# nsdumont/Semantic-Spiking-Neural-SLAM-2023

Hardware: AMD Instinct MI355X
Metric: sim-sec/wall-sec, SSP-SLAM ssp_dim=1015 10k PI neurons, 1/2/4/8 MI355X (higher is better)
Workload: dtype f32; 1 GPU; PathIntegration 2-D ssp_dim=1015 pi_n_neurons=10000/VCO (508 VCOs, 5080000 LIF neurons), configs[1]; eval_points_per_vco=4000, parallelism=1 GPU, build_cache=miss

## Files before the change

### include/ssn.h

```cpp
#ifndef SSN_H
#define SSN_H

#include <stdint.h>

#ifdef __cplusplus
extern "C" {
#endif

#define SSN_ABI_VERSION 10

enum ssn_status {
  SSN_OK = 0,
  SSN_EINVAL = -1,
  SSN_EHIP = -2,
  SSN_ERCCL = -3,
  SSN_ENOMEM = -4,
  SSN_EUNSUPPORTED = -5
};

enum ssn_dtype { SSN_F32 = 0, SSN_F64 = 1 };
enum ssn_buffer_kind { SSN_BUF_REAL = 0, SSN_BUF_I32 = 1, SSN_BUF_TAPS = 2 ,
                       SSN_BUF_DRIVES = 3  };
enum ssn_neuron { SSN_LIF = 0, SSN_LIFRATE = 1, SSN_RELU = 2 };

// ... 167 lines not shown

enum ssn_probe_kind {
  SSN_PROBE_PK_FMA = 0, SSN_PROBE_PK_MUL = 1, SSN_PROBE_PK_ADD = 2,
  SSN_PROBE_TRANS = 3,
  SSN_PROBE_FMA = 4, SSN_PROBE_ADD = 5,
  SSN_PROBE_DPP = 6, SSN_PROBE_MOV = 7, SSN_PROBE_READLANE = 8,
  SSN_PROBE_CNDMASK = 9, SSN_PROBE_OTHER = 10,
  SSN_PROBE_N_KINDS = 11
};
int ssn_probe_issue_rate(int32_t device, int32_t kind, int32_t waves_per_simd, int32_t iters,
                         double* ns_per_wave_instruction, double* shader_mhz);

int ssn_get_counters(ssn_sim* sim, ssn_counters* out);
int ssn_get_kernel_times(ssn_sim* sim, ssn_kernel_time* out, int32_t capacity);
int64_t ssn_n_steps(ssn_sim* sim);
int ssn_device_count(void);
const char* ssn_last_error(void);
const char* ssn_version(void);

#ifdef __cplusplus
}
#endif
#endif
```

### semantic-spiking-neural-slam-2023_amd/_lib.py

```python
import ctypes as C
import os

_HERE = os.path.dirname(os.path.abspath(__file__))
LIB_PATH = os.environ.get("SSN_HIP_LIB") or os.path.join(_HERE, "libssn_hip.so")

SSN_ABI_VERSION = 10
SSN_F32, SSN_F64 = 0, 1
SSN_BUF_REAL, SSN_BUF_I32, SSN_BUF_TAPS, SSN_BUF_DRIVES = 0, 1, 2, 3
NEURON_CODE = {"lif": 0, "lifrate": 1, "relu": 2}
OP_CODE = {"fill": 1, "table": 2, "axpy": 3, "matvec": 4, "lowpass": 5, "ensarray": 6, "neurons": 7,
           "pes": 8, "voja": 9, "cleanup": 10, "gate": 11, "lincomb": 12}
SSN_PLAN_NO_FUSED_CORE = 1
SSN_PLAN_NO_LIF_FAST = 2
SSN_PLAN_DENSE_DECODERS = 4
SSN_PLAN_NO_SPMV = 8
SSN_PLAN_SEPARATE_FINISH = 16
SSN_PLAN_NO_BLOCK_KERNEL = 128
SSN_PLAN_NO_FFT = 512
SSN_PLAN_SPMV_OWN_LIST = 1024
SSN_PLAN_NO_ITEM_BATCH = 4096
SSN_PLAN_ENS_PARTIALS = 8192
SSN_PLAN_NO_STAGE_BATCH = 262144
SSN_PLAN_NO_FACTORED_GRID = 524288
SSN_PLAN_NO_ROUNDS = 2097152
# ... 79 lines not shown
    "ssn_read_signal": (C.c_int, [C.c_void_p, C.c_int64, C.c_int64, C.c_void_p]),
    "ssn_write_signal": (C.c_int, [C.c_void_p, C.c_int64, C.c_int64, C.c_void_p]),
    "ssn_read_buffer": (C.c_int, [C.c_void_p, C.c_int32, C.c_void_p, C.c_int64]),
    "ssn_write_buffer": (C.c_int, [C.c_void_p, C.c_int32, C.c_void_p, C.c_int64]),
    "ssn_run_phase": (C.c_int, [C.c_void_p, C.c_int32]),
    "ssn_exchange_size": (C.c_int64, [C.c_void_p]),
    "ssn_cycle_steps": (C.c_int64, [C.c_void_p]),
    "ssn_exchange_pack": (C.c_int, [C.c_void_p, C.c_void_p]),
    "ssn_exchange_unpack": (C.c_int, [C.c_void_p, C.c_void_p]),
    "ssn_phase_async": (C.c_int, [C.c_void_p, C.c_int32, C.c_void_p, C.c_void_p]),
    "ssn_phase_sync": (C.c_int, [C.c_void_p, C.c_void_p]),
    "ssn_probe_issue_rate": (C.c_int, [C.c_int32, C.c_int32, C.c_int32, C.c_int32, C.POINTER(C.c_double), C.POINTER(C.c_double)]),
    "ssn_get_counters": (C.c_int, [C.c_void_p, C.POINTER(Counters)]),
    "ssn_get_kernel_times": (C.c_int, [C.c_void_p, C.POINTER(KernelTime), C.c_int32]),
    "ssn_n_steps": (C.c_int64, [C.c_void_p]),
    "ssn_device_count": (C.c_int, []),
    "ssn_last_error": (C.c_char_p, []),
    "ssn_version": (C.c_char_p, []),
}

_lib = None


def load():
    global _lib
    if _lib is not None:
        return _lib
    if not os.path.exists(LIB_PATH):
        raise ImportError(f"{LIB_PATH} not found: build it with `python -c 'import __graft_entry__ as g; g.build()'` "
                          "or `make -C semantic-spiking-neural-slam-2023_amd/csrc` (there is no CPU fallback)")
# ... 15 lines not shown
```

### semantic-spiking-neural-slam-2023_amd/csrc/ssn_host.hip

```cpp
#include <hip/hip_runtime.h>
#include <dlfcn.h>
#include <algorithm>
#include <climits>
#include <cmath>
#include <cstdarg>
#include <cstdio>
#include <cstdlib>
#include <cstring>
#include <memory>
#include <mutex>
#include <map>
#include <set>
#include <string>
#include <thread>
#include <vector>

#include "../../include/ssn.h"
#include "ssn_launch.hpp"

namespace {

__global__ void k_set_block(ssn::StepCtx* ctx, long long block_start) { ctx->block_start = block_start; }
__global__ void k_advance(ssn::StepCtx* ctx, long long n) { ctx->step += n; }

thread_local std::string g_err;

int fail(int code, const char* fmt, ...) {
  char buf[1024];
  va_list ap;
  va_start(ap, fmt);
  vsnprintf(buf, sizeof buf, fmt, ap);
  va_end(ap);
  g_err = buf;
  return code;
}

}
// ... 92 lines not shown
  X(REAL, lat_solo, "SSN_LAT_SOLO", 3.0, "balancer: latency of a gate / argmax body (us)")                                                        \
  X(OFF0, pes_fold, "SSN_PES_FOLD", true, "fold the filter of a PES rule's activities into the rule's body")                                      \
  X(ON1, phased_pes_fold, "SSN_PHASED_PES_FOLD", false, "... also in neuron-sharded plans")                                                       \
  X(OFF0, fuse_neurons, "SSN_FUSE_NEURONS", true, "neuron update of a dense population in the epilogue of its encoder product")                   \
  X(INT, fuse_min_rows, "SSN_FUSE_MIN_ROWS", 4097, "smallest population that is fused so (tests lower it)")                                       \
  X(OFF0, solo_chains, "SSN_SOLO_CHAINS", true, "serial chains of single-workgroup operators (RK_SOLO)")                                          \
  X(OFF0, phased_solo, "SSN_PHASED_SOLO", true, "... in neuron-sharded plans")                                                                    \
  X(ON1, solo_dft, "SSN_SOLO_DFT", false, "transforms as members of serial chains (measured slower)")                                             \
  X(REAL, solo_cap_us, "SSN_SOLO_CAP_US", 16.0, "longest serial chain in estimated microseconds")                                                 \
  X(LL, solo_max_len, "SSN_SOLO_MAX_LEN", 2048, "longest glue operator (elements) a single workgroup takes")                                      \
  X(OFF0, round_interleave, "SSN_ROUND_INTERLEAVE", true, "interleaved dispatch of a round's big grids behind its latency-bound head")            \
  X(OFF0, head_prio, "SSN_HEAD_PRIO", true, "raised wave priority for the head blocks of a round")                                                \
  X(PRESENT, phase2_sequential, "SSN_PHASE2_SEQUENTIAL", false, "sharded: phase 1 of a timestep and phase 0 of the next as two sets of rounds")   \
  X(INT, cycle_steps, "SSN_CYCLE_STEPS", 16, "sharded: timesteps pipelined over the exchange (2..64; 0 or 1: off)")                               \
  X(PRESENT, no_batch_reorder, "SSN_NO_BATCH_REORDER", false, "time-batched stages keep the builder's operator order")                            \
  X(PRESENT, no_zero_skip, "SSN_NO_ZERO_SKIP", false, "time-batched products are multiplied out even when their whole input is zero")

struct PlanOptions {
  struct Int3 { int v[3] = {0, 0, 0}; };
  static constexpr int UNSET = INT_MIN;
  enum Kind { K_PRESENT, K_OFF0, K_ON1, K_INT, K_LL, K_REAL, K_INT3 };
  typedef bool T_PRESENT; typedef bool T_OFF0; typedef bool T_ON1; typedef int T_INT; typedef long long T_LL; typedef double T_REAL; typedef Int3 T_INT3;

  int flags = 0;
#define X(kind, name, env, def, doc) T_##kind name = def;
  SSN_PLAN_KNOBS(X)
#undef X

  bool has(int bit) const { return (flags & bit) != 0; }

  static PlanOptions read(int flags) {
// ... 76 lines not shown
  virtual int reserve_probes(int64_t n) = 0;
  virtual int run_steps(int64_t n, int profile) = 0;
  virtual int run_phase(int phase) = 0;
  virtual int64_t exchange_size() = 0;
  virtual int64_t cycle_len() = 0;
  virtual int exchange_copy(void* buf, bool pack) = 0;
  virtual int phase_async(int phase, void* buf, hipStream_t ext) = 0;
  virtual int phase_sync(hipStream_t ext) = 0;
  virtual int read_probe(int id, double* dst, void* dst_dev, int64_t first, int64_t count) = 0;
  virtual int64_t probe_count(int id) = 0;
  virtual int rw_signal(int64_t off, int64_t count, double* dst, const double* src) = 0;
  virtual int rw_buffer(int id, double* dst, const double* src, int64_t count) = 0;
  virtual int counters(ssn_counters* out) = 0;
  virtual int kernel_times(ssn_kernel_time* out, int capacity) = 0;
  virtual int64_t n_steps() = 0;
};

namespace {

template <typename T>
struct Sim final : ssn_sim {
  using MOp = ssn::MicroOp<T>;
  static constexpr int VW = 16 / sizeof(T);

  struct TapSet;
  struct DriveSet;
  struct Item {
    int type = IT_PROGRAM;
    int op_begin = 0, op_count = 0;
    ssn::EnsArgs<T> ens;
// ... 22 lines not shown
  hipStream_t stream = nullptr;
  hipStream_t copy_stream = nullptr;
  double* up_stage = nullptr;
  int64_t up_cap = 0;
  void* dl_stage = nullptr;
  int64_t dl_cap = 0;
  std::mutex dl_mutex;
  int64_t n_sig = 0;
  T* sig = nullptr;
  std::vector<double> sig_init;
  std::vector<Buf> bufs;
  std::vector<Item> items;
  std::vector<void*> owned;
  T* bsig = nullptr;
  int block = 0;
  bool core_empty = false;
  const PlanOptions opt;
  bool fused_core = false;
  bool fused_defer = false;
  ssn::FinishArgs<T> fin_begin, fin_flush;
  bool fused_block = false;
  ssn::BlockArgs<T> blk;
  struct TapSet { std::vector<ssn_tap_desc> list; int* d_tab = nullptr; double amp = 0.0; };
  std::map<int, TapSet> tap_sets;
  struct DriveSet { ssn_drive_desc rec; std::vector<int32_t> src; int* d_tab = nullptr; int* d_tab_rows = nullptr; };
  std::map<int, DriveSet> drive_sets;
  std::set<int> sparse_w;
  std::set<int> learned_w;
  std::vector<std::pair<int64_t, std::pair<int*, int*>>> spike_lists;
  std::vector<int64_t> seg_spikes;
// ... 540 lines not shown
    }
    pslots.assign(m->n_probes, ssn::ProbeSlot{nullptr, 1, 0, 0});
    probe_store.resize((size_t)m->n_probes);
    for (int i = 0; i < m->n_probes; ++i) pslots[i].every = probes[i].every;
    CHK(dupload(&d_pslots, pslots));
    exchange.assign(m->exchange, m->exchange + (m->n_exchange > 0 ? m->n_exchange : 0));
    phased = !exchange.empty();
    for (auto& r : exchange) CHK(check_range(r.lo, r.hi - r.lo, "exchange"));
    bool has_batched_stage = false;
    for (int i = 0; i < m->n_ops; ++i) has_batched_stage = has_batched_stage || m->ops[i].stage != 1;
    for (auto& p : probes) has_batched_stage = has_batched_stage || p.stage != 1;
    batched_mask.assign((size_t)n_sig, 0);
    if (has_batched_stage && phased) return fail(SSN_EINVAL, "a neuron-sharded model is stepped whole (build it unstaged)");
    if (has_batched_stage) {
      block = m->block_steps > 0 ? m->block_steps : ((int64_t)1025 * n_sig * (int64_t)sizeof(T) <= (256ll << 20) ? 1024 : 256);
      CHK(dmalloc(&bsig, (int64_t)(block + 1) * n_sig * (int64_t)sizeof(T)));
      CHK(init_bsig());
      pre_to_core.assign(m->pre_to_core, m->pre_to_core + m->n_pre_to_core);
      core_to_post.assign(m->core_to_post, m->core_to_post + m->n_core_to_post);
      for (auto& r : pre_to_core) CHK(check_range(r.lo, r.hi - r.lo, "pre->core boundary"));
      for (auto& r : core_to_post) CHK(check_range(r.lo, r.hi - r.lo, "core->post boundary"));
    }
    steps_per_graph = m->steps_per_graph != 0 ? m->steps_per_graph : ((block == 0 || block % 64 == 0) ? 64 : 16);
    if (steps_per_graph > 128) return fail(SSN_EINVAL, "steps_per_graph %d: at most 128 (a glue block carries its timestep offset in 8 signed bits)", steps_per_graph);
    CHK(drive_tables());
    CHK(plan(m));
    CHK(capture());
    HIPCHK(hipStreamSynchronize(stream));
    return SSN_OK;
  }

  ssn::NeuronParams<T> neuron_params(int64_t type, const double* f) const {
// ... 418 lines not shown
      if (hipGetDeviceProperties(&prop, device) == hipSuccess) n_cu = prop.multiProcessorCount;
      if (opt.block_split_cus != PlanOptions::UNSET) n_cu = opt.block_split_cus;
      const int64_t n_ens = eo.i[2];
      for (int cand : {4, 2}) {
        if (K * cand <= n_cu && n_ens / cand >= 1024) { split_P = cand; break; }
      }
      { const int q = opt.block_split; if (q == 1 || q == 2 || q == 4 || q == 8) split_P = q; }
      if (split_P > 1) n_member = (int)(((n_ens + split_P - 1) / split_P + 3) / 4 * 4);
    }
    if (defer && !drv && !opt.has(SSN_PLAN_NO_BLOCK_KERNEL) && ens_fast(eo) && (sizeof(T) == 8 || (dt <= 0.05 * eo.f[0] && eo.f[1] >= dt)) &&
        ssn::ens_block_supported<T>((int)din, (int)dout, split_P > 1 ? n_member : (int)eo.i[2], opt.block_variant.v, &blk_threads, &blk_tpb, &blk_npt, &blk_lds)) {
      FilterTabs ft;
      CHK(filter_tables(ft, true));
      ssn::EnsArgs<T> ea;
      fill_ens_args(eo, taps, drv, ea);
      blk = ssn::BlockArgs<T>{};
      blk.enc = ea.enc; blk.bias = ea.bias; blk.dec = ea.dec; blk.S = ea.V;
      blk.xrows = bsig; blk.bsig = bsig; blk.sig = sig; blk.sig_w = sig;
      blk.didx = (const int*)bufs[eo.i[8]].d; blk.lp_state = ft.lp; blk.lp_a = ft.a; blk.lp_b = ft.b;
      blk.xrow = ft.xrow; blk.xalpha = ft.xalpha; blk.rowout = ft.ro;
      blk.n_sig = n_sig; blk.x_off = eo.i[0];
      blk.K = ea.K; blk.n = ea.n; blk.n_pad = ea.n_pad; blk.din = ea.din; blk.dout = ea.dout;
      blk.B = 0; blk.row0 = 1; blk.threads = blk_threads; blk.tpb = blk_tpb; blk.npt = blk_npt; blk.enc_lds = blk_lds;
      blk.dec_neuron_major = ea.fast == 1 ? 1 : 0;
      blk.np = ea.np;
      blk.P = split_P; blk.n_member = n_member; blk.xslots = nullptr; blk.xerr = nullptr;
      {
        unsigned long long* d_ss = nullptr;
        CHK(dzeros(&d_ss, 2));
        blk.slot_stats = d_ss;
// ... 367 lines not shown
    bool first_probe = true;
    for (size_t p = 0; p < probes.size(); ++p) {
      if (probes[p].stage != 1) {
        ssn::BatchOp<T> b{};
        b.bsig = bsig; b.n_sig = n_sig; b.kind = ssn::M_PROBE; b.src = probes[p].src; b.len = probes[p].width; b.p0 = d_pslots + p;
        post_ops.push_back(b);
        continue;
      }
      MOp op{};
      op.kind = ssn::M_PROBE; op.src = probes[p].src; op.len = probes[p].width; op.p0 = d_pslots + p;
      push_micro(op, -2, first_probe);
      first_probe = false;
    }
    optimise_batch(pre_ops);
    optimise_batch(post_ops);
    if (!fused) {
      MOp end{};
      end.kind = ssn::M_STEP_END;
      push_micro(end, -3, false);
    }
    force_barrier = true;
    flush();
    for (auto& it : items) if (it.phase < 0) it.phase = cur_phase;
    if (phased && cur_phase != 1) return fail(SSN_EINVAL, "a model with exchange ranges needs operators of phase 1");
    if (best_item >= 0) {
      items[best_item].dominant = true;
      const ssn::EnsArgs<T>& a = items[best_item].ens;
      dom_units = (int64_t)a.K * a.n;
      dom_bytes = (double)dom_units * (a.din + a.dout + 5) * sizeof(T);
    }
// ... 1104 lines not shown
      if (it.type == IT_PROGRAM) {
        for (const MOp& op : programs[(size_t)item_prog[(size_t)prog_i]]) micro_access(acc[i], op);
        ++prog_i;
      } else if (it.type == IT_VECOPS) {
        for (const MOp& op : vecops_host) micro_access(acc[i], op);
      } else {
        item_access(acc[i], it);
      }
    }
    item_deps.assign(items.size(), {});
    for (size_t i = 0; i < items.size(); ++i)
      for (size_t j = 0; j < i; ++j)
        if (hazard(acc[i], acc[j])) item_deps[i].push_back((int)j);
  }

  int init_bsig() {
    if (!bsig) return SSN_OK;
    CHK(upload(sig_init.data(), bsig, 1, n_sig, n_sig));
    for (int r = 1; r <= block; ++r)
      HIPCHK(hipMemcpyAsync(bsig + (size_t)r * n_sig, bsig, (size_t)n_sig * sizeof(T), hipMemcpyDeviceToDevice, stream));
    HIPCHK(hipStreamSynchronize(stream));
    return SSN_OK;
  }

  static bool batch_elementwise(const ssn::BatchOp<T>& o) { return kind_is(o.kind, MK_BATCH_EW); }
  static bool batch_writes(const ssn::BatchOp<T>& o) { return kind_is(o.kind, MK_BATCH_W); }
  static bool batch_reads(const ssn::BatchOp<T>& o) { return kind_is(o.kind, MK_BATCH_R); }
  static long long batch_read_len(const ssn::BatchOp<T>& o) { return kind_is(o.kind, MK_BATCH_PRODUCT) ? o.cols : o.len; }
  static int batch_hazard(const ssn::BatchOp<T>& a, const ssn::BatchOp<T>& b) {
    auto ov = [](long long x, long long xl, long long y, long long yl) { return x < y + yl && y < x + xl; };
    int kind = 0;
    auto pair = [&](long long x, long long xl, long long y, long long yl, bool prev) {
      if (!ov(x, xl, y, yl)) return;
      kind = std::max(kind, (x == y && !prev) ? 1 : 2);
    };
// ... 53 lines not shown
      if (!out.empty() && level[k] == last_level && o.kind == ssn::M_LOWPASS && out.back().kind == ssn::M_LOWPASS && out.back().a == o.a && out.back().b == o.b &&
          out.back().src_prev == o.src_prev && out.back().dst + out.back().len == o.dst && out.back().src + out.back().len == o.src) {
        out.back().len += o.len;
        continue;
      }
      out.push_back(o);
      last_level = level[k];
    }
    if (opt.debug_plan) {
      fprintf(stderr, "[ssn] time-batched stage: %zu operators -> %zu\n", ops.size(), out.size());
      for (const Op& o : out) fprintf(stderr, "[ssn]   batch op kind %d dst %lld src %lld len %lld cols %d prev %d\n", o.kind, (long long)o.dst, (long long)o.src, (long long)o.len, o.cols, o.src_prev);
    }
    ops.swap(out);
  }

  hipError_t run_batch(std::vector<ssn::BatchOp<T>>& ops, int B, int64_t step0) {
    auto elementwise = [](const ssn::BatchOp<T>& o) { return batch_elementwise(o); };
    std::vector<char> zero((size_t)n_sig, 0);
    const bool track = !opt.no_zero_skip;
    auto all_zero = [&](long long lo, long long n) { for (long long q = lo; q < lo + n; ++q) if (!zero[(size_t)q]) return false; return n > 0; };
    auto set_zero = [&](long long lo, long long n, bool v) { for (long long q = lo; q < lo + n; ++q) zero[(size_t)q] = v ? 1 : 0; };
    auto note = [&](const ssn::BatchOp<T>& o) {
      if (!track) return;
      switch (o.kind) {
        case ssn::M_TABLE: {
          bool z = false;
          for (size_t id = 0; id < table_dst.size() && id < table_idx_host.size(); ++id)
            if (table_dst[id].second > 0 && table_dst[id].first == o.dst && table_dst[id].second == o.len) z = table_is_zero((int)id, B, step0);
          set_zero(o.dst, o.len, z); break;
        }
        case ssn::M_FILL: set_zero(o.dst, o.len, o.a == T(0)); break;
        case ssn::M_AXPY_SET: set_zero(o.dst, o.len, !o.src_prev && all_zero(o.src, o.len)); break;
        case ssn::M_AXPY_INC: if (o.src_prev || !all_zero(o.src, o.len)) set_zero(o.dst, o.len, false); break;
        case ssn::M_PROBE: break;
        default: set_zero(o.dst, o.len, false); break;
      }
    };
    for (size_t i = 0; i < ops.size();) {
      ops[i].B = B; ops[i].step0 = step0;
      if (elementwise(ops[i]) && !opt.has(SSN_PLAN_NO_STAGE_BATCH)) {
        ssn::BatchOpList<T> l{};
        l.op[0] = ops[i];
        l.count = 1;
        size_t j = i + 1;
        for (; j < ops.size() && l.count < ssn::MAX_BATCH_OPS && elementwise(ops[j]); ++j) {
          ops[j].B = B; ops[j].step0 = step0;
          bool clash = false;
          for (int q = 0; q < l.count; ++q) clash = clash || batch_hazard(l.op[q], ops[j]) == 2;
          if (clash) break;
          l.op[l.count++] = ops[j];
        }
        if (l.count > 1) {
          hipError_t e = ssn::launch_batch_elementwise<T>(stream, l);
          if (e != hipSuccess) return e;
          for (int q = 0; q < l.count; ++q) note(l.op[q]);
          i = j;
          continue;
        }
      }
      if (track && kind_is(ops[i].kind, MK_BATCH_PRODUCT) && !ops[i].src_prev && all_zero(ops[i].src, ops[i].cols)) {
        ++batch_skipped;
        if (ops[i].kind == ssn::M_MATVEC_SET) {
          hipError_t e = hipMemset2DAsync(bsig + n_sig + ops[i].dst, (size_t)n_sig * sizeof(T), 0, (size_t)ops[i].len * sizeof(T), (size_t)B, stream);
          if (e != hipSuccess) return e;
          set_zero(ops[i].dst, ops[i].len, true);
        }
        ++i;
        continue;
      }
      hipError_t e = ssn::launch_batch_op<T>(stream, ops[i]);
      if (e != hipSuccess) return e;
      note(ops[i]);
      ++i;
    }
    return hipSuccess;
  }

  bool table_is_zero(int id, int B, int64_t step0) const {
    const ssn::TableSlot& t = tables[(size_t)id];
    const std::vector<int32_t>& ix = table_idx_host[(size_t)id];
    for (int64_t st = step0; st < step0 + B; ++st) {
      const int64_t rel = st - t.first_step;
      if (rel >= 0 && rel < (int64_t)ix.size() && ix[(size_t)rel] >= 0) return false;
    }
    return true;
  }
// ... 322 lines not shown
    Timing tm;
    tm.level = profile;
    if (profile) {
      const size_t per_step = profile == 2 ? items.size() + (round_mode ? launch_list.size() : 0) : (size_t)std::max(1, n_dom);
      const size_t need = fused_block ? (size_t)(2 * (n / std::max(1, block) + 2)) : (size_t)(2 * n * (int)per_step);
      if (need > 400000) return fail(SSN_EINVAL, "profile run too long (%lld steps): at most 200000 timed launches", (long long)n);
      while (ev_pool.size() < need) {
        hipEvent_t ev;
        HIPCHK(hipEventCreate(&ev));
        ev_pool.push_back(ev);
      }
    }
    HIPCHK(hipEventRecord(ev_run0, stream));
    int64_t done = 0;
    while (done < n) {
      const int64_t B = bsig ? std::min<int64_t>(block, n - done) : (n - done);
      const int64_t step0 = steps_done + done;
      if (bsig) {
        hipLaunchKernelGGL(k_set_block, dim3(1), dim3(1), 0, stream, d_ctx, (long long)step0);
        HIPCHK(hipGetLastError());
        HIPCHK(run_batch(pre_ops, (int)B, step0));
      }
      if (fused_defer) HIPCHK(ssn::launch_ens_finish<T>(stream, fin_begin));
      if (fused_block) {
        const bool timed = profile && B == block && tm.used + 2 <= ev_pool.size();
        blk.B = (int)B;
        if (blk.P > 1)
          HIPCHK(hipMemsetD32Async((hipDeviceptr_t)blk.xslots, (int)ssn::BLOCK_XCHG_SENTINEL, (size_t)3 * blk.K * 64, stream));
        if (timed) HIPCHK(hipEventRecord(ev_pool[tm.used], stream));
        HIPCHK(ssn::launch_ens_block<T>(stream, blk));
        if (timed) { HIPCHK(hipEventRecord(ev_pool[tm.used + 1], stream)); tm.used += 2; }
        HIPCHK(advance_clock(B));
      } else if (core_empty) {
        HIPCHK(advance_clock(B));
      } else if (profile) {
        int64_t s = 0;
        if (profile == 2 && round_mode && !graph_list.empty())
          for (; s + steps_per_graph <= B; s += steps_per_graph) {
            HIPCHK(launch_seq(graph_list, &tm));
            HIPCHK(advance_clock(steps_per_graph));
          }
        for (; s < B; ++s) {
          HIPCHK(launch_seq(launch_list, &tm));
          if (fused_defer) HIPCHK(advance_clock(1));
        }
      } else {
        int64_t left = B;
        if (step_graph.exec)
          for (; left >= steps_per_graph; left -= steps_per_graph) HIPCHK(hipGraphLaunch(step_graph.exec, stream));
        if (left > 0) HIPCHK(launch_steps((int)left, true));
      }
      if (fused_defer) HIPCHK(ssn::launch_ens_finish<T>(stream, fin_flush));
      if (bsig) {
        HIPCHK(run_batch(post_ops, (int)B, step0));
        HIPCHK(hipMemcpyAsync(bsig, bsig + (size_t)B * n_sig, (size_t)n_sig * sizeof(T), hipMemcpyDeviceToDevice, stream));
      }
      done += B;
    }
    HIPCHK(hipEventRecord(ev_run1, stream));
    HIPCHK(hipStreamSynchronize(stream));
    for (size_t j = 0; j < tm.used; j += 2) {
      float ms = 0.f;
      HIPCHK(hipEventElapsedTime(&ms, ev_pool[j], ev_pool[j + 1]));
      if (profile == 2) {
        const int ty = tm.types[j / 2];
        type_ms[ty] += ms;
        type_launches[ty] += 1;
        if (item_ms.size() != items.size() + round_launches.size()) { item_ms.assign(items.size() + round_launches.size(), 0.0); item_n.assign(items.size() + round_launches.size(), 0); }
        item_ms[(size_t)tm.items[j / 2]] += ms; item_n[(size_t)tm.items[j / 2]] += 1;
        continue;
      }
      dom_ms += ms;
// ... 208 lines not shown
                                              "k_argmax_partial", "k_round", "", "", ""};
    int n = 0;
    for (int t = 0; t < N_ITEM_TYPES; ++t) {
      if (!type_launches[t]) continue;
      if (n < capacity) {
        snprintf(out[n].name, sizeof out[n].name, "%s", names[t]);
        out[n].launches = type_launches[t];
        out[n].ms_total = type_ms[t];
      }
      ++n;
    }
    return n;
  }

  int64_t n_steps() override { return steps_done; }
};

template <typename T>
int create_sim(const ssn_model_desc* desc, ssn_sim** out) {
  auto s = std::make_unique<Sim<T>>(desc);
  int rc = s->create(desc);
  if (rc != SSN_OK) return rc;
  *out = s.release();
  return SSN_OK;
}

}

extern "C" {

// ... 71 lines not shown
  return sim->exchange_copy(dst_dev, true);
}
int ssn_exchange_unpack(ssn_sim* sim, const void* src_dev) {
  if (!sim || !src_dev) return fail(SSN_EINVAL, "null argument");
  return sim->exchange_copy(const_cast<void*>(src_dev), false);
}
int ssn_phase_async(ssn_sim* sim, int32_t phase, void* exchange_buf, void* hip_stream) {
  return sim ? sim->phase_async(phase, exchange_buf, (hipStream_t)hip_stream) : fail(SSN_EINVAL, "null simulator");
}
int ssn_phase_sync(ssn_sim* sim, void* hip_stream) { return sim ? sim->phase_sync((hipStream_t)hip_stream) : fail(SSN_EINVAL, "null simulator"); }
int ssn_get_kernel_times(ssn_sim* sim, ssn_kernel_time* out, int32_t capacity) {
  if (!sim || (!out && capacity > 0) || capacity < 0) return fail(SSN_EINVAL, "null argument");
  return sim->kernel_times(out, capacity);
}
int64_t ssn_n_steps(ssn_sim* sim) { return sim ? sim->n_steps() : -1; }
int ssn_device_count(void) {
  int n = 0;
  return hipGetDeviceCount(&n) == hipSuccess ? n : 0;
}
const char* ssn_last_error(void) { return g_err.c_str(); }
const char* ssn_version(void) { return "libssn_hip 0.10 (gfx950, ABI 10)"; }

}
```

### semantic-spiking-neural-slam-2023_amd/csrc/ssn_kernels.hpp

```cpp
#pragma once
#include <hip/hip_runtime.h>
#include <stdint.h>
#include <algorithm>
#include "ssn_launch.hpp"

namespace ssn {

template <typename T> struct VecT;
template <> struct VecT<float>  { using type = float4;  static constexpr int W = 4; };
template <> struct VecT<double> { using type = double2; static constexpr int W = 2; };

__device__ inline float  expm1_(float x)  { return expm1f(x); }
__device__ inline double expm1_(double x) { return expm1(x); }
__device__ inline float  log1p_(float x)  { return log1pf(x); }
__device__ inline double log1p_(double x) { return log1p(x); }

template <typename T> struct LifMath;
template <> struct LifMath<double> {
  const double tau_rc;
  __device__ explicit LifMath(const NeuronParams<double>& p) : tau_rc(p.tau_rc) {}
  __device__ double decay(double delta) const { return expm1(-delta / tau_rc); }
  __device__ double spike_time_term(double V, double J) const { return log1p(-(V - 1.0) / (J - 1.0)); }
};
template <> struct LifMath<float> {
// ... 1980 lines not shown
}

template <typename T>
hipError_t launch_gemm_nt(hipStream_t s, const T* A, int lda, const T* Wm, int ldw, T* C, int ldc, int M, int N, int K, int splits) {
  if constexpr (sizeof(T) == 4) {
    const int kper = ((K + splits - 1) / splits + 31) / 32 * 32;
    hipLaunchKernelGGL((k_gemm_nt_mfma_f32<32>), dim3((unsigned)((N + 63) / 64), (unsigned)((M + 63) / 64), (unsigned)((K + kper - 1) / kper)),
                       dim3(256), 0, s, A, lda, Wm, ldw, C, ldc, M, N, K, kper);
    return hipGetLastError();
  } else {
    return hipErrorInvalidValue;
  }
}

template <typename T>
hipError_t launch_batch_op(hipStream_t s, const BatchOp<T>& o) {
  if (o.B <= 0 || o.len <= 0) return hipSuccess;
  if (o.kind == M_LOWPASS) {
    if constexpr (sizeof(T) == 4) {
      if (o.B >= 256) {
        hipLaunchKernelGGL((kb_lowpass_chunked<32, 32>), dim3((unsigned)((o.len + 31) / 32)), dim3(1024), 0, s, o);
        return hipGetLastError();
      }
    }
    hipLaunchKernelGGL((kb_lowpass<T>), dim3((unsigned)((o.len + 63) / 64)), dim3(64), 0, s, o);
  } else if ((o.kind == M_MATVEC_INC || o.kind == M_MATVEC_SET) && sizeof(T) == 4 && o.cols >= 64 && o.len >= 32 && o.B >= 32) {
    if constexpr (sizeof(T) == 4)
      hipLaunchKernelGGL((kb_gemm_mfma_f32<32>), dim3((unsigned)((o.len + 63) / 64), (unsigned)((o.B + 63) / 64)), dim3(1024), 0, s, o);
  } else if (o.kind == M_MATVEC_INC || o.kind == M_MATVEC_SET) {
    hipLaunchKernelGGL((kb_gemm<T>), dim3((unsigned)((o.len + 31) / 32), (unsigned)((o.B + 31) / 32)), dim3(256), 0, s, o);
  } else {
    const long long total = (long long)o.B * o.len;
    const unsigned grid = (unsigned)std::min<long long>((total + 255) / 256, 4096);
    hipLaunchKernelGGL((kb_elementwise<T>), dim3(grid), dim3(256), 0, s, o);
  }
  return hipGetLastError();
}

template <typename T>
__global__ void k_convert_in(const double* __restrict__ src, T* __restrict__ dst, int64_t rows, int64_t cols, int64_t ld) {
  const int64_t i = (int64_t)blockIdx.x * 256 + threadIdx.x;
// ... 34 lines not shown
  template bool ens_block_supported<T>(int, int, int, const int*, int*, int*, int*, int*);                             \
  template hipError_t launch_ensarray<T>(hipStream_t, const EnsArgs<T>&);                                    \
  template hipError_t launch_ensarray_batch<T>(hipStream_t, const EnsBatch<T>&, int);                        \
  template hipError_t launch_dec_pack<T>(hipStream_t, const T*, T*, int, int, int, int, int, int);           \
  template hipError_t launch_state_unpack<T>(hipStream_t, const T*, T*, int64_t, int, T);                    \
  template hipError_t launch_program<T>(hipStream_t, const MicroOp<T>*, const ProgDesc*, int, T*, StepCtx*); \
  template hipError_t launch_vecops<T>(hipStream_t, const MicroOp<T>*, int, int, T*, const StepCtx*);        \
  template hipError_t launch_ens_finish<T>(hipStream_t, const FinishArgs<T>&);                               \
  template hipError_t launch_matvec<T>(hipStream_t, const MatvecBatch<T>&, int);            \
  template hipError_t launch_matvec_ordered<T>(hipStream_t, const T*, const T*, T*, int, int, int);         \
  template hipError_t launch_spmv_partial<T>(hipStream_t, const SpmvBatch<T>&, int); \
  template hipError_t launch_transpose<T>(hipStream_t, const T*, T*, int, int, int, int);                   \
  template hipError_t launch_neurons<T>(hipStream_t, const NeuronsBatch<T>&, int); \
  template hipError_t launch_pes<T>(hipStream_t, T*, const T*, const T*, int, int, int, T);                 \
  template hipError_t launch_voja<T>(hipStream_t, T*, const T*, const T*, const T*, const T*, int, int, int, T); \
  template hipError_t launch_batch_op<T>(hipStream_t, const BatchOp<T>&);                                   \
  template hipError_t launch_grid_lhs<T>(hipStream_t, const T*, const T*, int, T*, int, int, int);          \
  template hipError_t launch_argmax_partial<T>(hipStream_t, const T*, long long, T*, int, int);             \
  template hipError_t launch_gemm_nt<T>(hipStream_t, const T*, int, const T*, int, T*, int, int, int, int, int); \
  template hipError_t launch_batch_elementwise<T>(hipStream_t, const BatchOpList<T>&);                      \
  template hipError_t launch_convert_in<T>(hipStream_t, const double*, T*, int64_t, int64_t, int64_t);      \
  template hipError_t launch_convert_out<T>(hipStream_t, const T*, double*, int64_t, int64_t, int64_t);      \
  template hipError_t launch_round<T>(hipStream_t, const RoundArgs<T>&, int, size_t);

}
```

### semantic-spiking-neural-slam-2023_amd/csrc/ssn_launch.hpp

```cpp
#pragma once
#include <hip/hip_runtime.h>
#include <stdint.h>
#include <atomic>

namespace ssn {

inline hipError_t set_max_dynamic_lds_once(const void* fn, int bytes, std::atomic<uint64_t>& done) {
  int dev = 0;
  hipError_t e = hipGetDevice(&dev);
  if (e != hipSuccess) return e;
  const uint64_t bit = 1ull << (dev & 63);
  if (done.load(std::memory_order_acquire) & bit) return hipSuccess;
  e = hipFuncSetAttribute(fn, hipFuncAttributeMaxDynamicSharedMemorySize, bytes);
  if (e == hipSuccess) done.fetch_or(bit, std::memory_order_release);
  return e;
}

template <typename T>
struct NeuronParams {
  int type;
  T dt, tau_rc, tau_ref, min_voltage;
};

struct StepCtx;
// ... 239 lines not shown
template <typename T> hipError_t launch_state_unpack(hipStream_t, const T* src, T* out, int64_t n, int want_refractory, T r_offset);
template <typename T> hipError_t launch_ens_finish(hipStream_t, const FinishArgs<T>&);
template <typename T> hipError_t launch_dft(hipStream_t, const DftBatch&, int count);
template <typename T> hipError_t launch_ens_block(hipStream_t, const BlockArgs<T>&);
template <typename T> bool ens_block_supported(int din, int dout, int n, const int want[3], int* threads, int* tpb, int* npt, int* enc_lds);
template <typename T> hipError_t launch_program(hipStream_t, const MicroOp<T>* ops, const ProgDesc* progs, int n_progs, T* sig, StepCtx* ctx);
template <typename T> hipError_t launch_vecops(hipStream_t, const MicroOp<T>* ops, int n_ops, int wgs, T* sig, const StepCtx* ctx);
template <typename T> hipError_t launch_matvec(hipStream_t, const MatvecBatch<T>&, int count);
template <typename T> hipError_t launch_matvec_ordered(hipStream_t, const T* Wt, const T* x, T* y, int rows, int cols, int ldt);
template <typename T> hipError_t launch_transpose(hipStream_t, const T* src, T* dst, int rows, int cols, int ld, int ldt);
template <typename T> hipError_t launch_spmv_partial(hipStream_t, const SpmvBatch<T>&, int count);
template <typename T> hipError_t launch_neurons(hipStream_t, const NeuronsBatch<T>&, int count);
template <typename T> hipError_t launch_pes(hipStream_t, T* W, const T* err, const T* act, int rows, int cols, int ld, T kappa);
template <typename T> hipError_t launch_voja(hipStream_t, T* E, const T* spk, const T* key, const T* learn, const T* scale,
                                            int rows, int cols, int ld, T lr_dt);
template <typename T> hipError_t launch_batch_op(hipStream_t, const BatchOp<T>&);
template <typename T> hipError_t launch_argmax_partial(hipStream_t, const T* sims, long long n, T* out, int P, int nsplit);
template <typename T> hipError_t launch_grid_lhs(hipStream_t, const T* X, const T* E, int lde, T* A, int lda, int na, int K);
template <typename T> hipError_t launch_gemm_nt(hipStream_t, const T* A, int lda, const T* Wm, int ldw, T* C, int ldc, int M, int N, int K, int splits);
template <typename T> hipError_t launch_convert_in(hipStream_t, const double* src, T* dst, int64_t rows, int64_t cols, int64_t ld);
template <typename T> hipError_t launch_convert_out(hipStream_t, const T* src, double* dst, int64_t rows, int64_t cols, int64_t ld);

}
```

### semantic-spiking-neural-slam-2023_amd/simulator.py

```python
import ctypes as C
import os
import time

import numpy as np

from . import _lib
from ._lib import (
    SSN_PLAN_NO_FUSED_CORE, SSN_PLAN_NO_LIF_FAST, SSN_PLAN_DENSE_DECODERS, SSN_PLAN_NO_SPMV, SSN_PLAN_SEPARATE_FINISH,
    SSN_PLAN_NO_BLOCK_KERNEL, SSN_PLAN_NO_FFT, SSN_PLAN_SPMV_OWN_LIST, SSN_PLAN_NO_ITEM_BATCH, SSN_PLAN_ENS_PARTIALS,
    SSN_PLAN_NO_STAGE_BATCH, SSN_PLAN_NO_FACTORED_GRID, SSN_PLAN_NO_ROUNDS, SSN_PLAN_ENS_OWN_LAUNCH,
    SSN_PLAN_NO_PIPELINE, SSN_PLAN_NO_BALANCE, SSN_PLAN_NO_CUTS, SSN_PLAN_NO_CHAINS, SSN_PLAN_BLUESTEIN_FFT,
    SSN_PLAN_FOUR_STEP_FFT, SSN_PLAN_SPLIT_BLOCK,
    PLAN_FLAGS)
from . import frontend as fe
from .builder import BuiltModel, build


class SimulationData(dict):

    def __init__(self, sim):
        super().__init__()
        self._sim = sim

    def __getitem__(self, key):
# ... 584 lines not shown
        out = np.empty(shape, dtype=np.float64)
        self._check(self._lib.ssn_read_buffer(self._h, buffer_id, out.ctypes.data, out.size))
        return out

    def write_buffer(self, buffer_id, values):
        v = np.ascontiguousarray(values, dtype=np.float64)
        self._check(self._lib.ssn_write_buffer(self._h, buffer_id, v.ctypes.data, v.size))

    def read_probe_device(self, probe, dst_ptr, first, count):
        kind, j, p = self._probe_index[probe]
        self._check(self._lib.ssn_read_probe_device(self._h, j, C.c_void_p(dst_ptr), first, count))

    def counters(self):
        c = _lib.Counters()
        self._check(self._lib.ssn_get_counters(self._h, C.byref(c)))
        return {f: getattr(c, f) for f, _ in c._fields_}

    def run_phase(self, phase):
        if phase == 3:
            self._cycle_segment(lambda: self._lib.ssn_run_phase(self._h, 3))
            return
        if phase not in (0, 1, 2):
            raise fe.SimulationError(f"run_phase({phase}): 0, 1, 2 or 3")
        if phase in (0, 2) and self._prepared_until < self.n_steps + (1 if phase == 0 else 2):
            raise fe.SimulationError("neuron-sharded model: call prepare(n_steps) before stepping")
        self._check(self._lib.ssn_run_phase(self._h, int(phase)))
        if phase >= 1:
            self.n_steps += 1
            self._uncollected = True

    def cycle_steps(self):
# ... 67 lines not shown
```

Baseline: 361.9 sim-sec/wall-sec.

## Let several time blocks share one run of the time-batched stages

Adds a stage_span option so the pre/post time-batched stages can process several blocks of timesteps in a single run, with the block kernel iterating over row offsets inside the enlarged staging buffer. Zero-skip tracking becomes per segment, and lowpass is launched per segment. It also replaces the per-row device copies that initialise the staging buffer with a single spreading kernel. Spanning is meant to cut per-block launch overhead and enlarge GEMM batches, at the cost of more memory and hazard checks, but the default span is 1.

```diff
diff --git a/include/ssn.h b/include/ssn.h
--- a/include/ssn.h
+++ b/include/ssn.h
@@ -205,6 +205,7 @@
 int ssn_get_counters(ssn_sim* sim, ssn_counters* out);
 int ssn_get_kernel_times(ssn_sim* sim, ssn_kernel_time* out, int32_t capacity);
 int64_t ssn_n_steps(ssn_sim* sim);
+int64_t ssn_stage_span(ssn_sim* sim);
 int ssn_device_count(void);
 const char* ssn_last_error(void);
 const char* ssn_version(void);
diff --git a/semantic-spiking-neural-slam-2023_amd/_lib.py b/semantic-spiking-neural-slam-2023_amd/_lib.py
--- a/semantic-spiking-neural-slam-2023_amd/_lib.py
+++ b/semantic-spiking-neural-slam-2023_amd/_lib.py
@@ -117,6 +117,7 @@
     "ssn_get_counters": (C.c_int, [C.c_void_p, C.POINTER(Counters)]),
     "ssn_get_kernel_times": (C.c_int, [C.c_void_p, C.POINTER(KernelTime), C.c_int32]),
     "ssn_n_steps": (C.c_int64, [C.c_void_p]),
+    "ssn_stage_span": (C.c_int64, [C.c_void_p]),
     "ssn_device_count": (C.c_int, []),
     "ssn_last_error": (C.c_char_p, []),
     "ssn_version": (C.c_char_p, []),
diff --git a/semantic-spiking-neural-slam-2023_amd/csrc/ssn_host.hip b/semantic-spiking-neural-slam-2023_amd/csrc/ssn_host.hip
--- a/semantic-spiking-neural-slam-2023_amd/csrc/ssn_host.hip
+++ b/semantic-spiking-neural-slam-2023_amd/csrc/ssn_host.hip
@@ -21,6 +21,11 @@
 namespace {
 
 __global__ void k_set_block(ssn::StepCtx* ctx, long long block_start) { ctx->block_start = block_start; }
+template <typename T>
+__global__ __launch_bounds__(256) void k_spread_row0(T* buf, long long n, long long rows) {
+  const long long total = n * rows;
+  for (long long e = (long long)blockIdx.x * 256 + threadIdx.x; e < total; e += (long long)gridDim.x * 256) buf[n + e] = buf[e % n];
+}
 __global__ void k_advance(ssn::StepCtx* ctx, long long n) { ctx->step += n; }
 
 thread_local std::string g_err;
@@ -143,7 +148,8 @@
   X(PRESENT, phase2_sequential, "SSN_PHASE2_SEQUENTIAL", false, "sharded: phase 1 of a timestep and phase 0 of the next as two sets of rounds")   \
   X(INT, cycle_steps, "SSN_CYCLE_STEPS", 16, "sharded: timesteps pipelined over the exchange (2..64; 0 or 1: off)")                               \
   X(PRESENT, no_batch_reorder, "SSN_NO_BATCH_REORDER", false, "time-batched stages keep the builder's operator order")                            \
-  X(PRESENT, no_zero_skip, "SSN_NO_ZERO_SKIP", false, "time-batched products are multiplied out even when their whole input is zero")
+  X(PRESENT, no_zero_skip, "SSN_NO_ZERO_SKIP", false, "time-batched products are multiplied out even when their whole input is zero")           \
+  X(INT, stage_span, "SSN_STAGE_SPAN", UNSET, "whole-block plan: blocks that share one run of the time-batched stages (1: a run per block)")
 
 struct PlanOptions {
   struct Int3 { int v[3] = {0, 0, 0}; };
@@ -250,6 +256,7 @@
   virtual int counters(ssn_counters* out) = 0;
   virtual int kernel_times(ssn_kernel_time* out, int capacity) = 0;
   virtual int64_t n_steps() = 0;
+  virtual int64_t stage_span_blocks() = 0;
 };
 
 namespace {
@@ -302,6 +309,7 @@
   std::vector<void*> owned;
   T* bsig = nullptr;
   int block = 0;
+  int stage_span = 1;
   bool core_empty = false;
   const PlanOptions opt;
   bool fused_core = false;
@@ -872,8 +880,7 @@
     if (has_batched_stage && phased) return fail(SSN_EINVAL, "a neuron-sharded model is stepped whole (build it unstaged)");
     if (has_batched_stage) {
       block = m->block_steps > 0 ? m->block_steps : ((int64_t)1025 * n_sig * (int64_t)sizeof(T) <= (256ll << 20) ? 1024 : 256);
-      CHK(dmalloc(&bsig, (int64_t)(block + 1) * n_sig * (int64_t)sizeof(T)));
-      CHK(init_bsig());
+      CHK(size_bsig(1));
       pre_to_core.assign(m->pre_to_core, m->pre_to_core + m->n_pre_to_core);
       core_to_post.assign(m->core_to_post, m->core_to_post + m->n_core_to_post);
       for (auto& r : pre_to_core) CHK(check_range(r.lo, r.hi - r.lo, "pre->core boundary"));
@@ -1322,6 +1329,7 @@
       CHK(filter_tables(ft, true));
       ssn::EnsArgs<T> ea;
       fill_ens_args(eo, taps, drv, ea);
+      if (split_P == 1 && wanted_stage_span() > 1) CHK(size_bsig(wanted_stage_span()));
       blk = ssn::BlockArgs<T>{};
       blk.enc = ea.enc; blk.bias = ea.bias; blk.dec = ea.dec; blk.S = ea.V;
       blk.xrows = bsig; blk.bsig = bsig; blk.sig = sig; blk.sig_w = sig;
@@ -1719,6 +1727,7 @@
     }
     optimise_batch(pre_ops);
     optimise_batch(post_ops);
+    if (stage_span > 1 && !(span_safe(pre_ops, &post_ops) && span_safe(post_ops, nullptr))) stage_span = 1;
     if (!fused) {
       MOp end{};
       end.kind = ssn::M_STEP_END;
@@ -2853,11 +2862,33 @@
         if (hazard(acc[i], acc[j])) item_deps[i].push_back((int)j);
   }
 
+  static constexpr int STAGE_SPAN_DEFAULT = 1;
+  static constexpr int64_t STAGE_SPAN_BUDGET = 512ll << 20;
+  int wanted_stage_span() const {
+    const int64_t want = opt.stage_span != PlanOptions::UNSET ? opt.stage_span : STAGE_SPAN_DEFAULT;
+    const int64_t fit = (STAGE_SPAN_BUDGET / (n_sig * (int64_t)sizeof(T)) - 1) / block;
+    return (int)std::max<int64_t>(1, std::min(want, fit));
+  }
+
+  int size_bsig(int span) {
+    if (bsig) {
+      owned.erase(std::find(owned.begin(), owned.end(), (void*)bsig));
+      HIPCHK(hipFree(bsig));
+      device_bytes -= (int64_t)(stage_span * (int64_t)block + 1) * n_sig * (int64_t)sizeof(T);
+      bsig = nullptr;
+    }
+    stage_span = span;
+    CHK(dmalloc(&bsig, (int64_t)(stage_span * (int64_t)block + 1) * n_sig * (int64_t)sizeof(T)));
+    return init_bsig();
+  }
+
   int init_bsig() {
     if (!bsig) return SSN_OK;
     CHK(upload(sig_init.data(), bsig, 1, n_sig, n_sig));
-    for (int r = 1; r <= block; ++r)
-      HIPCHK(hipMemcpyAsync(bsig + (size_t)r * n_sig, bsig, (size_t)n_sig * sizeof(T), hipMemcpyDeviceToDevice, stream));
+    const long long rows = (long long)stage_span * block;
+    const unsigned grid = (unsigned)std::min<long long>((rows * n_sig + 255) / 256, 4096);
+    hipLaunchKernelGGL((k_spread_row0<T>), dim3(grid), dim3(256), 0, stream, bsig, (long long)n_sig, rows);
+    HIPCHK(hipGetLastError());
     HIPCHK(hipStreamSynchronize(stream));
     return SSN_OK;
   }
@@ -2941,37 +2972,63 @@
     ops.swap(out);
   }
 
-  hipError_t run_batch(std::vector<ssn::BatchOp<T>>& ops, int B, int64_t step0) {
+  static bool span_safe(const std::vector<ssn::BatchOp<T>>& ops, const std::vector<ssn::BatchOp<T>>* after) {
+    auto ov = [](long long x, long long xl, long long y, long long yl) { return x < y + yl && y < x + xl; };
+    for (size_t k = 0; k < ops.size(); ++k) {
+      const ssn::BatchOp<T>& o = ops[k];
+      auto written_later = [&](long long lo, long long n) {
+        for (size_t q = k + 1; q < ops.size(); ++q) if (batch_writes(ops[q]) && ov(lo, n, ops[q].dst, ops[q].len)) return true;
+        if (after) for (const ssn::BatchOp<T>& w : *after) if (batch_writes(w) && ov(lo, n, w.dst, w.len)) return true;
+        return false;
+      };
+      if (o.src_prev && batch_reads(o) && written_later(o.src, batch_read_len(o))) return false;
+      if (o.kind == ssn::M_LOWPASS && written_later(o.dst, o.len)) return false;
+    }
+    return true;
+  }
+
+  hipError_t run_batch(std::vector<ssn::BatchOp<T>>& ops, int rows, int64_t step0) {
     auto elementwise = [](const ssn::BatchOp<T>& o) { return batch_elementwise(o); };
-    std::vector<char> zero((size_t)n_sig, 0);
+    const int nseg = (rows + block - 1) / block;
+    auto seg_rows = [&](int s) { return std::min(block, rows - s * block); };
+    auto part = [&](const ssn::BatchOp<T>& o, int r0, int nr) {
+      ssn::BatchOp<T> q = o;
+      q.bsig = o.bsig + (size_t)r0 * n_sig; q.B = nr; q.step0 = step0 + r0;
+      return q;
+    };
+    std::vector<char> zero((size_t)nseg * (size_t)n_sig, 0);
     const bool track = !opt.no_zero_skip;
-    auto all_zero = [&](long long lo, long long n) { for (long long q = lo; q < lo + n; ++q) if (!zero[(size_t)q]) return false; return n > 0; };
-    auto set_zero = [&](long long lo, long long n, bool v) { for (long long q = lo; q < lo + n; ++q) zero[(size_t)q] = v ? 1 : 0; };
+    auto all_zero = [&](int s, long long lo, long long n) {
+      for (long long q = lo; q < lo + n; ++q) if (!zero[(size_t)s * (size_t)n_sig + (size_t)q]) return false;
+      return n > 0;
+    };
+    auto set_zero = [&](int s, long long lo, long long n, bool v) { for (long long q = lo; q < lo + n; ++q) zero[(size_t)s * (size_t)n_sig + (size_t)q] = v ? 1 : 0; };
     auto note = [&](const ssn::BatchOp<T>& o) {
       if (!track) return;
-      switch (o.kind) {
-        case ssn::M_TABLE: {
-          bool z = false;
-          for (size_t id = 0; id < table_dst.size() && id < table_idx_host.size(); ++id)
-            if (table_dst[id].second > 0 && table_dst[id].first == o.dst && table_dst[id].second == o.len) z = table_is_zero((int)id, B, step0);
-          set_zero(o.dst, o.len, z); break;
-        }
-        case ssn::M_FILL: set_zero(o.dst, o.len, o.a == T(0)); break;
-        case ssn::M_AXPY_SET: set_zero(o.dst, o.len, !o.src_prev && all_zero(o.src, o.len)); break;
-        case ssn::M_AXPY_INC: if (o.src_prev || !all_zero(o.src, o.len)) set_zero(o.dst, o.len, false); break;
-        case ssn::M_PROBE: break;
-        default: set_zero(o.dst, o.len, false); break;
-      }
+      for (int s = 0; s < nseg; ++s)
+        switch (o.kind) {
+          case ssn::M_TABLE: {
+            bool z = false;
+            for (size_t id = 0; id < table_dst.size() && id < table_idx_host.size(); ++id)
+              if (table_dst[id].second > 0 && table_dst[id].first == o.dst && table_dst[id].second == o.len) z = table_is_zero((int)id, seg_rows(s), step0 + (int64_t)s * block);
+            set_zero(s, o.dst, o.len, z); break;
+          }
+          case ssn::M_FILL: set_zero(s, o.dst, o.len, o.a == T(0)); break;
+          case ssn::M_AXPY_SET: set_zero(s, o.dst, o.len, !o.src_prev && all_zero(s, o.src, o.len)); break;
+          case ssn::M_AXPY_INC: if (o.src_prev || !all_zero(s, o.src, o.len)) set_zero(s, o.dst, o.len, false); break;
+          case ssn::M_PROBE: break;
+          default: set_zero(s, o.dst, o.len, false); break;
+        }
     };
     for (size_t i = 0; i < ops.size();) {
-      ops[i].B = B; ops[i].step0 = step0;
+      ops[i].B = rows; ops[i].step0 = step0;
       if (elementwise(ops[i]) && !opt.has(SSN_PLAN_NO_STAGE_BATCH)) {
         ssn::BatchOpList<T> l{};
         l.op[0] = ops[i];
         l.count = 1;
         size_t j = i + 1;
         for (; j < ops.size() && l.count < ssn::MAX_BATCH_OPS && elementwise(ops[j]); ++j) {
-          ops[j].B = B; ops[j].step0 = step0;
+          ops[j].B = rows; ops[j].step0 = step0;
           bool clash = false;
           for (int q = 0; q < l.count; ++q) clash = clash || batch_hazard(l.op[q], ops[j]) == 2;
           if (clash) break;
@@ -2985,18 +3042,36 @@
           continue;
         }
       }
-      if (track && kind_is(ops[i].kind, MK_BATCH_PRODUCT) && !ops[i].src_prev && all_zero(ops[i].src, ops[i].cols)) {
-        ++batch_skipped;
-        if (ops[i].kind == ssn::M_MATVEC_SET) {
-          hipError_t e = hipMemset2DAsync(bsig + n_sig + ops[i].dst, (size_t)n_sig * sizeof(T), 0, (size_t)ops[i].len * sizeof(T), (size_t)B, stream);
-          if (e != hipSuccess) return e;
-          set_zero(ops[i].dst, ops[i].len, true);
+      if (kind_is(ops[i].kind, MK_BATCH_PRODUCT)) {
+        const ssn::BatchOp<T>& o = ops[i];
+        auto skipped = [&](int s) { return track && !o.src_prev && all_zero(s, o.src, o.cols); };
+        for (int s = 0; s < nseg;) {
+          const bool skip = skipped(s);
+          int e = s + 1;
+          while (e < nseg && skipped(e) == skip && ssn::batch_product_mfma(o, seg_rows(e)) == ssn::batch_product_mfma(o, seg_rows(s))) ++e;
+          const int r0 = s * block, nr = std::min(rows, e * block) - r0;
+          hipError_t err = hipSuccess;
+          if (!skip) err = ssn::launch_batch_op<T>(stream, part(o, r0, nr), seg_rows(s));
+          else if (o.kind == ssn::M_MATVEC_SET)
+            err = hipMemset2DAsync(bsig + (size_t)(r0 + 1) * n_sig + o.dst, (size_t)n_sig * sizeof(T), 0, (size_t)o.len * sizeof(T), (size_t)nr, stream);
+          if (err != hipSuccess) return err;
+          if (skip) batch_skipped += e - s;
+          if (!skip || o.kind == ssn::M_MATVEC_SET)
+            for (int q = s; q < e; ++q) set_zero(q, o.dst, o.len, skip);
+          s = e;
         }
         ++i;
         continue;
       }
-      hipError_t e = ssn::launch_batch_op<T>(stream, ops[i]);
-      if (e != hipSuccess) return e;
+      if (ops[i].kind == ssn::M_LOWPASS) {
+        for (int s = 0; s < nseg; ++s) {
+          hipError_t e = ssn::launch_batch_op<T>(stream, part(ops[i], s * block, seg_rows(s)));
+          if (e != hipSuccess) return e;
+        }
+      } else {
+        hipError_t e = ssn::launch_batch_op<T>(stream, ops[i]);
+        if (e != hipSuccess) return e;
+      }
       note(ops[i]);
       ++i;
     }
@@ -3349,48 +3424,51 @@
     HIPCHK(hipEventRecord(ev_run0, stream));
     int64_t done = 0;
     while (done < n) {
-      const int64_t B = bsig ? std::min<int64_t>(block, n - done) : (n - done);
+      const int64_t R = bsig ? std::min<int64_t>((int64_t)stage_span * block, n - done) : (n - done);
       const int64_t step0 = steps_done + done;
       if (bsig) {
         hipLaunchKernelGGL(k_set_block, dim3(1), dim3(1), 0, stream, d_ctx, (long long)step0);
         HIPCHK(hipGetLastError());
-        HIPCHK(run_batch(pre_ops, (int)B, step0));
+        HIPCHK(run_batch(pre_ops, (int)R, step0));
       }
       if (fused_defer) HIPCHK(ssn::launch_ens_finish<T>(stream, fin_begin));
       if (fused_block) {
-        const bool timed = profile && B == block && tm.used + 2 <= ev_pool.size();
-        blk.B = (int)B;
-        if (blk.P > 1)
-          HIPCHK(hipMemsetD32Async((hipDeviceptr_t)blk.xslots, (int)ssn::BLOCK_XCHG_SENTINEL, (size_t)3 * blk.K * 64, stream));
-        if (timed) HIPCHK(hipEventRecord(ev_pool[tm.used], stream));
-        HIPCHK(ssn::launch_ens_block<T>(stream, blk));
-        if (timed) { HIPCHK(hipEventRecord(ev_pool[tm.used + 1], stream)); tm.used += 2; }
-        HIPCHK(advance_clock(B));
+        for (int64_t r = 0; r < R; r += block) {
+          const int64_t B = std::min<int64_t>(block, R - r);
+          const bool timed = profile && B == block && tm.used + 2 <= ev_pool.size();
+          blk.row0 = (int)(1 + r); blk.B = (int)B;
+          if (blk.P > 1)
+            HIPCHK(hipMemsetD32Async((hipDeviceptr_t)blk.xslots, (int)ssn::BLOCK_XCHG_SENTINEL, (size_t)3 * blk.K * 64, stream));
+          if (timed) HIPCHK(hipEventRecord(ev_pool[tm.used], stream));
+          HIPCHK(ssn::launch_ens_block<T>(stream, blk));
+          if (timed) { HIPCHK(hipEventRecord(ev_pool[tm.used + 1], stream)); tm.used += 2; }
+          HIPCHK(advance_clock(B));
+        }
       } else if (core_empty) {
-        HIPCHK(advance_clock(B));
+        HIPCHK(advance_clock(R));
       } else if (profile) {
         int64_t s = 0;
         if (profile == 2 && round_mode && !graph_list.empty())
-          for (; s + steps_per_graph <= B; s += steps_per_graph) {
+          for (; s + steps_per_graph <= R; s += steps_per_graph) {
             HIPCHK(launch_seq(graph_list, &tm));
             HIPCHK(advance_clock(steps_per_graph));
           }
-        for (; s < B; ++s) {
+        for (; s < R; ++s) {
           HIPCHK(launch_seq(launch_list, &tm));
           if (fused_defer) HIPCHK(advance_clock(1));
         }
       } else {
-        int64_t left = B;
+        int64_t left = R;
         if (step_graph.exec)
           for (; left >= steps_per_graph; left -= steps_per_graph) HIPCHK(hipGraphLaunch(step_graph.exec, stream));
         if (left > 0) HIPCHK(launch_steps((int)left, true));
       }
       if (fused_defer) HIPCHK(ssn::launch_ens_finish<T>(stream, fin_flush));
       if (bsig) {
-        HIPCHK(run_batch(post_ops, (int)B, step0));
-        HIPCHK(hipMemcpyAsync(bsig, bsig + (size_t)B * n_sig, (size_t)n_sig * sizeof(T), hipMemcpyDeviceToDevice, stream));
-      }
-      done += B;
+        HIPCHK(run_batch(post_ops, (int)R, step0));
+        HIPCHK(hipMemcpyAsync(bsig, bsig + (size_t)R * n_sig, (size_t)n_sig * sizeof(T), hipMemcpyDeviceToDevice, stream));
+      }
+      done += R;
     }
     HIPCHK(hipEventRecord(ev_run1, stream));
     HIPCHK(hipStreamSynchronize(stream));
@@ -3629,6 +3707,7 @@
   }
 
   int64_t n_steps() override { return steps_done; }
+  int64_t stage_span_blocks() override { return stage_span; }
 };
 
 template <typename T>
@@ -3730,6 +3809,7 @@
   return sim->kernel_times(out, capacity);
 }
 int64_t ssn_n_steps(ssn_sim* sim) { return sim ? sim->n_steps() : -1; }
+int64_t ssn_stage_span(ssn_sim* sim) { return sim ? sim->stage_span_blocks() : -1; }
 int ssn_device_count(void) {
   int n = 0;
   return hipGetDeviceCount(&n) == hipSuccess ? n : 0;
diff --git a/semantic-spiking-neural-slam-2023_amd/csrc/ssn_kernels.hpp b/semantic-spiking-neural-slam-2023_amd/csrc/ssn_kernels.hpp
--- a/semantic-spiking-neural-slam-2023_amd/csrc/ssn_kernels.hpp
+++ b/semantic-spiking-neural-slam-2023_amd/csrc/ssn_kernels.hpp
@@ -2018,17 +2018,18 @@
 }
 
 template <typename T>
-hipError_t launch_batch_op(hipStream_t s, const BatchOp<T>& o) {
+hipError_t launch_batch_op(hipStream_t s, const BatchOp<T>& o, int pick_B) {
   if (o.B <= 0 || o.len <= 0) return hipSuccess;
+  if (pick_B <= 0) pick_B = o.B;
   if (o.kind == M_LOWPASS) {
     if constexpr (sizeof(T) == 4) {
-      if (o.B >= 256) {
+      if (pick_B >= 256) {
         hipLaunchKernelGGL((kb_lowpass_chunked<32, 32>), dim3((unsigned)((o.len + 31) / 32)), dim3(1024), 0, s, o);
         return hipGetLastError();
       }
     }
     hipLaunchKernelGGL((kb_lowpass<T>), dim3((unsigned)((o.len + 63) / 64)), dim3(64), 0, s, o);
-  } else if ((o.kind == M_MATVEC_INC || o.kind == M_MATVEC_SET) && sizeof(T) == 4 && o.cols >= 64 && o.len >= 32 && o.B >= 32) {
+  } else if ((o.kind == M_MATVEC_INC || o.kind == M_MATVEC_SET) && batch_product_mfma(o, pick_B)) {
     if constexpr (sizeof(T) == 4)
       hipLaunchKernelGGL((kb_gemm_mfma_f32<32>), dim3((unsigned)((o.len + 63) / 64), (unsigned)((o.B + 63) / 64)), dim3(1024), 0, s, o);
   } else if (o.kind == M_MATVEC_INC || o.kind == M_MATVEC_SET) {
@@ -2093,7 +2094,7 @@
   template hipError_t launch_neurons<T>(hipStream_t, const NeuronsBatch<T>&, int); \
   template hipError_t launch_pes<T>(hipStream_t, T*, const T*, const T*, int, int, int, T);                 \
   template hipError_t launch_voja<T>(hipStream_t, T*, const T*, const T*, const T*, const T*, int, int, int, T); \
-  template hipError_t launch_batch_op<T>(hipStream_t, const BatchOp<T>&);                                   \
+  template hipError_t launch_batch_op<T>(hipStream_t, const BatchOp<T>&, int);                                 \
   template hipError_t launch_grid_lhs<T>(hipStream_t, const T*, const T*, int, T*, int, int, int);          \
   template hipError_t launch_argmax_partial<T>(hipStream_t, const T*, long long, T*, int, int);             \
   template hipError_t launch_gemm_nt<T>(hipStream_t, const T*, int, const T*, int, T*, int, int, int, int, int); \
diff --git a/semantic-spiking-neural-slam-2023_amd/csrc/ssn_launch.hpp b/semantic-spiking-neural-slam-2023_amd/csrc/ssn_launch.hpp
--- a/semantic-spiking-neural-slam-2023_amd/csrc/ssn_launch.hpp
+++ b/semantic-spiking-neural-slam-2023_amd/csrc/ssn_launch.hpp
@@ -277,7 +277,8 @@
 template <typename T> hipError_t launch_pes(hipStream_t, T* W, const T* err, const T* act, int rows, int cols, int ld, T kappa);
 template <typename T> hipError_t launch_voja(hipStream_t, T* E, const T* spk, const T* key, const T* learn, const T* scale,
                                             int rows, int cols, int ld, T lr_dt);
-template <typename T> hipError_t launch_batch_op(hipStream_t, const BatchOp<T>&);
+template <typename T> hipError_t launch_batch_op(hipStream_t, const BatchOp<T>&, int pick_B = 0);
+template <typename T> inline bool batch_product_mfma(const BatchOp<T>& o, int B) { return sizeof(T) == 4 && o.cols >= 64 && o.len >= 32 && B >= 32; }
 template <typename T> hipError_t launch_argmax_partial(hipStream_t, const T* sims, long long n, T* out, int P, int nsplit);
 template <typename T> hipError_t launch_grid_lhs(hipStream_t, const T* X, const T* E, int lde, T* A, int lda, int na, int K);
 template <typename T> hipError_t launch_gemm_nt(hipStream_t, const T* A, int lda, const T* Wm, int ldw, T* C, int ldc, int M, int N, int K, int splits);
diff --git a/semantic-spiking-neural-slam-2023_amd/simulator.py b/semantic-spiking-neural-slam-2023_amd/simulator.py
--- a/semantic-spiking-neural-slam-2023_amd/simulator.py
+++ b/semantic-spiking-neural-slam-2023_amd/simulator.py
@@ -622,7 +622,9 @@
     def counters(self):
         c = _lib.Counters()
         self._check(self._lib.ssn_get_counters(self._h, C.byref(c)))
-        return {f: getattr(c, f) for f, _ in c._fields_}
+        out = {f: getattr(c, f) for f, _ in c._fields_}
+        out["stage_span"] = int(self._lib.ssn_stage_span(self._h))
+        return out
 
     def run_phase(self, phase):
         if phase == 3:
```

Result: no change. 360.7 sim-sec/wall-sec (-0.3%).
